# yitian97/SDformerFlow

Measured on AMD Instinct MI355X. Metric: event-frames/sec fwd (1x10x2x288x384), higher is better.
Workload: dtype f16x2; 1 GPU; BASELINE configs[1]: MS_SpikingformerFlowNet_en4 forward, batch 1 per GPU, 10-bin 288x384 voxel, neuron=lif; a step = one forward of one sample; 2 HIP streams per GPU, each replaying the HIP graph of one launch sequence that carries 10 independent batch-1 forwards of different voxels (replicas: every flow map bit-equal to a separate batch-1 forward, asserted by --full runs); one process per GPU; in_flight=2, replicas_per_launch=10, samples_in_flight=20, hip_graph=True, weight_planes=2

## Files before the change

### sdformerflow_amd/csrc/spike_conv_wres.hip

```cpp
#include "spike_mm.h"
#include "switches.h"

#ifdef SDF_STAMP
__device__ unsigned long long g_wres_stamp[32];
#define STAMP(var) var = __builtin_readcyclecounter()
#define STAMP_ADD(acc, a, b) acc += (b) - (a)
#else
#define STAMP(var)
#define STAMP_ADD(acc, a, b)
#endif

namespace sdfmm {
namespace {

constexpr int TH = 8, TW = 16;
constexpr int HH = TH + 2, HWID = TW + 2;
constexpr int NB = 32;
constexpr uint32_t INV = 0x80000000u;

typedef __attribute__((ext_vector_type(4))) uint32_t u32x4;

__device__ __forceinline__ __amdgpu_buffer_rsrc_t make_rsrc(const void* p) {
  return __builtin_amdgcn_make_buffer_rsrc(const_cast<void*>(p), 0, (int)INV, 0x00020000);
}
// ... 340 lines not shown
  static constexpr int RCH = HW8 * CIN16;
  static constexpr int CPL = (HH8 + 1) / 2;
  static_assert(RCH <= 128, "a halo row must fit the 128 lanes of a half group");
  static_assert((PS / 4) % 8 == 4 && (WP / 4) % 8 == 4, "pitches must be 4 x odd dwords");
  static_assert(S2 || CIN % 32 == 0, "stride 1: K steps of 32 must not straddle taps");
  static_assert(!S2 || RB == 1, "stride 2: one row block per wave");
  static_assert(KH == 1 || S2, "channel passes: stride-2 form only");
  static constexpr int step_off(int ks) {
    constexpr int n = CIN16;
    if (ks < 3 * n) return (ks / n) * RPB + (ks % n) * 16;
    if (ks < 4 * n) return XE * PS + (ks - 3 * n) * 16;
    return 2 * RPB + XE * PS + (ks - 4 * n) * 32;
  }
  static constexpr int step_base(int ks) { return ks < 3 * CIN16 ? 0 : (ks < 4 * CIN16 ? 1 : 2); }
  static __device__ __forceinline__ int slot(int kc) {
    constexpr int n = CIN16;
    const int tap = kc / (n * KH), cg = kc - tap * (n * KH), hf = cg / n, c = cg - hf * n, ky = tap / 3, kx = tap - 3 * ky;
    const int base = 2 * KS * hf;
    if (kx != 1) return base + 2 * (ky * n + c) + (kx >> 1);
    if (ky < 2) return base + 2 * (3 * n + c) + ky;
    return base + 2 * 4 * n + c;
  }
};

template <int TT, int CIN16, int RB, int NGRP, bool S2 = false, int KH = 1, bool SPK = false>
__global__ __launch_bounds__(256 * NGRP) void spike_conv_wres_i8_kernel(GemmParams P, const float* __restrict__ col_scale) {
  static_assert(!SPK || TT > 0, "spikes-only: a fused-neuron form");
  using G = GeoI8<CIN16, RB, S2, KH>;
  constexpr int ST = S2 ? 2 : 1;
  constexpr int CING = G::CING;
  constexpr bool EARLY = KH > 1;
  constexpr bool SPIKE = TT > 0;
  const int T = SPIKE ? P.d.sn_T : 1;
  constexpr int CIN = G::CIN, K = G::K, PS = G::PS, RPB = G::RPB, WP = G::WP, TH8 = G::TH8, TW8 = G::TW8;
  constexpr int W_BYTES = 3 * NB * WP;
  constexpr int PAR = 2 * NB * 4;
  constexpr int NT = 256 * NGRP;
  static_assert(W_BYTES + NGRP * G::HALO + PAR + 64 <= 160 * 1024, "LDS budget");
  __shared__ __attribute__((aligned(16))) uint8_t smem[W_BYTES + NGRP * G::HALO + PAR + 64];
  uint8_t* W_s = smem;
  float* par_s = reinterpret_cast<float*>(smem + W_BYTES + NGRP * G::HALO);
  uint32_t* cnt = reinterpret_cast<uint32_t*>(smem + W_BYTES + NGRP * G::HALO + PAR);

  const SdfSpikeGemmDesc& d = P.d;
  const int H = P.cv.OH, W = P.cv.OW;
  const int Hin = P.cv.H, Win = P.cv.W;
  const int tid = threadIdx.x;
  const int wave = __builtin_amdgcn_readfirstlane(tid >> 6), lane = tid & 63;
  const int grp = wave >> 2, cw = wave & 3;
  const int gl = tid & 255;
  const int N = d.N;
  const bool has_res = !SPK && !(S2 && SPIKE) && d.resid != nullptr;
  const bool memb = !SPK && (!SPIKE || d.out != nullptr);
  const int ohw = H * W;
  const int pm = SPIKE ? (int)(d.pos_inner / ohw) : 1, pso = SPIKE ? (int)(d.pos_ostride / ohw) : 0;
  const int tstep = SPIKE ? (int)(d.t_stride / ohw) : 0;
  const bool lif_fast = SPIKE && d.sn_kind == SDF_LIF && d.soft_reset != 0 && P.inv_tau != 0.f;
  const bool soft = d.soft_reset != 0;

  if (tid < 2 * NGRP) cnt[tid] = 0;

  const int tiles_x = (W + TW8 - 1) / TW8, tiles_img = tiles_x * ((H + TH8 - 1) / TH8);
  const int Gd = gridDim.x;
  int wg = blockIdx.x;
  if ((Gd & 7) == 0) wg = (wg & 7) * (Gd >> 3) + (wg >> 3);
  int t_begin, n_my;
  if (P.cb_inner) {
    const int nr = Gd / P.tiles_n, r = wg / P.tiles_n, cbw = wg - r * P.tiles_n;
    const int base = P.tiles_m / nr, rem = P.tiles_m % nr;
    t_begin = cbw * P.tiles_m + r * base + (r < rem ? r : rem);
    n_my = base + (r < rem ? 1 : 0);
  } else {
    const int nitems = P.ntiles;
    const int base = nitems / Gd, rem = nitems % Gd;
    t_begin = wg * base + (wg < rem ? wg : rem);
    n_my = base + (wg < rem ? 1 : 0);
  }

  const int hhalf = gl >> 7, hj = gl & 127;
  const bool hj_ok = hj < G::RCH;
  const int hpx = (hj_ok ? hj : 0) / CIN16, hc16 = (hj_ok ? hj : 0) - hpx * CIN16;
  const uint32_t h_lds0 = (uint32_t)(hhalf * RPB + (S2 ? (hpx & 1) * G::XE * PS + (hpx >> 1) * PS : hpx * PS) + hc16 * 16);
  const int h_rel0 = ((hhalf - 1) * Win + (hpx - 1)) * CING + hc16 * 16;
  const __amdgpu_buffer_rsrc_t A_rs = make_rsrc(d.A);
  u32x4 hreg[G::CPL];
  auto halo_load = [&](int img, int y0, int x0, int hf) __attribute__((always_inline)) {
    const uint32_t org = (uint32_t)(((img * Hin + ST * y0) * Win + ST * x0) * CING + hf * CIN) + (uint32_t)h_rel0;
    const bool xok = hj_ok && (unsigned)(ST * x0 + hpx - 1) < (unsigned)Win;
#pragma unroll
    for (int i = 0; i < G::CPL; ++i) {
      const int hy = 2 * i + hhalf;
      const bool ok = xok && hy < G::HH8 && (unsigned)(ST * y0 + hy - 1) < (unsigned)Hin;
      hreg[i] = __builtin_amdgcn_raw_buffer_load_b128(A_rs, ok ? org + (uint32_t)(2 * i * Win * CING) : INV, 0, 0);
    }
  };
  uint8_t* H_s = smem + W_BYTES + grp * G::HALO;
  auto halo_store = [&]() __attribute__((always_inline)) {
#pragma unroll
    for (int i = 0; i < G::CPL; ++i)
      if (hj_ok && 2 * i + hhalf < G::HH8) *reinterpret_cast<u32x4*>(H_s + h_lds0 + 2 * i * RPB) = hreg[i];
  };
  auto item_decode = [&](int item, int& cb, int& img0, int& y0, int& x0) __attribute__((always_inline)) {
    cb = item / P.tiles_m;
    const int rt = item - cb * P.tiles_m;
    const int im = rt / tiles_img, tl = rt - im * tiles_img;
    const int ty = tl / tiles_x, tx = tl - ty * tiles_x;
    img0 = SPIKE ? (im / pm) * pso + im % pm : im; y0 = ty * TH8; x0 = tx * TW8;
  };

  int ln = lane;
  asm volatile("" : "+v"(ln));
  const int l31 = ln & 31, lh = ln >> 5;
  const uint32_t a_lane = S2 ? (uint32_t)(2 * (2 * cw + (l31 >> 4)) * RPB + (l31 & 15) * PS)
                              : (uint32_t)((2 * RB * cw + (l31 >> 4)) * RPB + (l31 & 15) * PS + 16 * lh);
  const uint32_t a_base[3] = {a_lane + (uint32_t)(lh * PS), a_lane + (uint32_t)(lh * RPB), a_lane + (uint32_t)(lh * 16)};
  const uint32_t w_lane = (uint32_t)(l31 * WP + 16 * lh);
  const __amdgpu_buffer_rsrc_t out_rs = make_rsrc(d.out), res_rs = make_rsrc(d.resid), sp_rs = make_rsrc(d.out_spike);

  uint32_t nstep = 0;
  int seg_begin = 0;
#ifdef SDF_STAMP
  unsigned long long s0 = 0, s1 = 0, s2 = 0, s3 = 0, s4 = 0, s5 = 0, a_issue = 0, a_wait = 0, a_mfma = 0, a_epi = 0, a_hand = 0, a_wload = 0;
  const unsigned long long kstart = __builtin_readcyclecounter(), rstart = __builtin_amdgcn_s_memrealtime();
#endif
  while (seg_begin < n_my) {
    int cb, img0, y0, x0;
    item_decode(t_begin + seg_begin, cb, img0, y0, x0);
    int seg_end = (cb + 1) * P.tiles_m - t_begin;
    if (seg_end > n_my) seg_end = n_my;
    const int n0 = cb * NB;
    STAMP(s0);
    __syncthreads();
    {
      constexpr int KC16 = K / 16;
      constexpr int WCH = 3 * NB * KC16;
      const __amdgpu_buffer_rsrc_t W_rs = __builtin_amdgcn_make_buffer_rsrc(const_cast<uint16_t*>(d.Wp), 0, 3 * N * K, 0x00020000);
      constexpr int WB = 6, NBATCH = (WCH + NT * WB - 1) / (NT * WB);
      int tl = tid;
      asm volatile("" : "+v"(tl));
#pragma unroll 1
      for (int b = 0; b < NBATCH; ++b) {
        u32x4 wv[WB];
#pragma unroll
        for (int i = 0; i < WB; ++i) {
          const int c = tl + NT * (b * WB + i);
          const int cc = c < WCH ? c : 0;
          const int row = cc / KC16, kc = cc - row * KC16;
          const int dg = row / NB, n = row - dg * NB;
          wv[i] = __builtin_amdgcn_raw_buffer_load_b128(W_rs, c < WCH ? (uint32_t)((dg * N + n0 + n) * K + kc * 16) : INV, 0, 0);
        }
#pragma unroll
        for (int i = 0; i < WB; ++i) {
          const int c = tl + NT * (b * WB + i);
          const int cc = c < WCH ? c : 0;
          const int row = cc / KC16, kc = cc - row * KC16;
          if (c < WCH) *reinterpret_cast<u32x4*>(W_s + row * WP + (S2 ? G::slot(kc) : kc) * 16) = wv[i];
        }
      }
      if (S2 && (G::NP & 1) && tid < 3 * NB) {
        u32x4 z; z.x = z.y = z.z = z.w = 0u;
#pragma unroll
        for (int hf = 0; hf < KH; ++hf) *reinterpret_cast<u32x4*>(W_s + tid * WP + (2 * G::KS * hf + G::NP) * 16) = z;
      }
      if (tid < 2 * NB) {
        const int which = tid / NB, n = tid - which * NB;
        const float sc = col_scale[n0 + n];
        par_s[tid] = which == 0 ? (d.alpha ? d.alpha[n0 + n] * sc : sc) : (d.alpha ? d.beta[n0 + n] : 0.f);
      }
    }
    __syncthreads();
    STAMP(s1); STAMP_ADD(a_wload, s0, s1);

    int it = seg_begin + grp;
    if (it < seg_end) {
      item_decode(t_begin + it, cb, img0, y0, x0);
      halo_load(img0, y0, x0, 0);
      if (nstep) wait_ge(&cnt[NGRP + grp], 4 * nstep);
      halo_store();
      signal(&cnt[grp], lane);
    }
    for (; it < seg_end; it += NGRP) {
      item_decode(t_begin + it, cb, img0, y0, x0);
      float vmem[SPIKE ? 16 * RB : 1];
      if (SPIKE) {
#pragma unroll
        for (int e = 0; e < 16 * RB; ++e) vmem[e] = soft ? 0.f : d.v_reset;
      }
#pragma unroll 1
      for (int t = 0; t < T; ++t) {
        STAMP(s0);
        const int img = img0 + t * tstep;
        const uint32_t ld4 = (uint32_t)d.ldo * 4u, col4 = (uint32_t)(n0 + 4 * lh) * 4u;
        const int ybase = y0 + 2 * RB * cw + (l31 >> 4), xbase = x0 + (l31 & 15);
        const uint32_t g00 = (uint32_t)((img * H + ybase) * W + xbase);
        auto row_g = [&](int rb, int q4) __attribute__((always_inline)) -> uint32_t {
          return (ybase + 2 * rb < H && xbase < W) ? g00 + (uint32_t)(2 * rb * W) : INV;
        };
        auto rowoff = [&](int rb, int q4) __attribute__((always_inline)) -> uint32_t {
          const uint32_t g = row_g(rb, q4);
          return g != INV ? g * ld4 + col4 + (uint32_t)(32 * q4) : INV;
        };
        float4 rs[RB][4];
#pragma unroll
        for (int rb = 0; rb < RB; ++rb)
#pragma unroll
          for (int q4 = 0; q4 < 4; ++q4) rs[rb][q4] = make_float4(0.f, 0.f, 0.f, 0.f);
        auto load_res = [&]() __attribute__((always_inline)) {
#pragma unroll
          for (int rb = 0; rb < RB; ++rb)
#pragma unroll
            for (int q4 = 0; q4 < 4; ++q4) rs[rb][q4] = buf_load16f(res_rs, rowoff(rb, q4));
        };
        constexpr bool RES_EARLY = !SPIKE || RB == 1;
        if (RES_EARLY && has_res) load_res();
        bool have_next = true;
        auto request_next = [&](int hf) __attribute__((always_inline)) {
          int ni = img, ny = y0, nx = x0, nhf = hf + 1;
          if (nhf == KH) {
            nhf = 0; ni = img0 + (t + 1) * tstep;
            if (t + 1 == T) {
              if (it + NGRP < seg_end) { int ncb; item_decode(t_begin + it + NGRP, ncb, ni, ny, nx); }
              else have_next = false;
            }
          }
          if (have_next) halo_load(ni, ny, nx, nhf);
        };
        auto hand_over = [&]() __attribute__((always_inline)) {
          if (have_next) {
            wait_ge(&cnt[NGRP + grp], 4 * nstep);
            halo_store();
            signal(&cnt[grp], lane);
          }
        };

        i32x16 acc[3][RB];
#pragma unroll
        for (int dg = 0; dg < 3; ++dg)
#pragma unroll
          for (int rb = 0; rb < RB; ++rb)
#pragma unroll
            for (int e = 0; e < 16; ++e) acc[dg][rb][e] = 0;
        constexpr int KS = G::KS;
        constexpr int PF = (RB == 1 && (NGRP == 2 || SPK)) ? 2 : 1;
#pragma unroll
        for (int hf = 0; hf < KH; ++hf) {
          ++nstep;
          if (EARLY) request_next(hf);
          STAMP(s1);
          wait_ge(&cnt[grp], 4 * nstep);
          STAMP(s2);
          i32x4 fa[PF + 1][RB], fb[PF + 1][3];
          auto frag = [&](int ks, int set) __attribute__((always_inline)) {
            if constexpr (S2) {
              fa[set][0] = *reinterpret_cast<const i32x4*>(H_s + a_base[G::step_base(ks)] + G::step_off(ks));
            } else {
              constexpr int C32 = CIN / 32;
              const int tap = ks / C32, c = ks - tap * C32;
              const int ky = tap / 3, kx = tap - 3 * ky;
#pragma unroll
              for (int rb = 0; rb < RB; ++rb)
                fa[set][rb] = *reinterpret_cast<const i32x4*>(H_s + a_lane + ((2 * rb + ky) * RPB + kx * PS + c * 32));
            }
#pragma unroll
            for (int dg = 0; dg < 3; ++dg)
              fb[set][dg] = *reinterpret_cast<const i32x4*>(W_s + w_lane + (dg * NB * WP + (hf * KS + ks) * 32));
          };
#pragma unroll
          for (int i = 0; i < PF; ++i) frag(i, i);
#pragma unroll
          for (int ks = 0; ks < KS; ++ks) {
            if (ks + PF < KS) frag(ks + PF, (ks + PF) % (PF + 1));
            __builtin_amdgcn_sched_barrier(0);
#pragma unroll
            for (int dg = 0; dg < 3; ++dg)
#pragma unroll
              for (int rb = 0; rb < RB; ++rb)
                acc[dg][rb] = __builtin_amdgcn_mfma_i32_32x32x32_i8(fb[ks % (PF + 1)][dg], fa[ks % (PF + 1)][rb], acc[dg][rb], 0, 0, 0);
            __builtin_amdgcn_sched_barrier(0);
          }
          signal(&cnt[NGRP + grp], lane);
          if (EARLY && hf + 1 < KH) hand_over();
        }
        STAMP(s3);

        if (!RES_EARLY && has_res) load_res();
        if (!EARLY) request_next(KH - 1);
#pragma unroll
        for (int rb = 0; rb < RB; ++rb) {
          float4 om[4];
#pragma unroll
          for (int q4 = 0; q4 < 4; ++q4) {
            __builtin_amdgcn_sched_barrier(0);
            float v[4];
#pragma unroll
            for (int j = 0; j < 4; ++j) {
              const int e = q4 * 4 + j;
              const int lo = acc[1][rb][e] * 256 + acc[0][rb][e];
              v[j] = __builtin_fmaf((float)acc[2][rb][e], 65536.f, (float)lo);
            }
            const float4 al4 = *reinterpret_cast<const float4*>(par_s + 8 * q4 + 4 * lh);
            const float4 be4 = *reinterpret_cast<const float4*>(par_s + NB + 8 * q4 + 4 * lh);
            float4 o;
            o.x = __builtin_fmaf(v[0], al4.x, be4.x) + rs[rb][q4].x; o.y = __builtin_fmaf(v[1], al4.y, be4.y) + rs[rb][q4].y;
            o.z = __builtin_fmaf(v[2], al4.z, be4.z) + rs[rb][q4].z; o.w = __builtin_fmaf(v[3], al4.w, be4.w) + rs[rb][q4].w;
            om[q4] = o;
            if (SPIKE) {
              const float xs[4] = {o.x, o.y, o.z, o.w};
              uint32_t pk = 0;
              if (lif_fast) {
#pragma unroll
                for (int j = 0; j < 4; ++j) {
                  float& vm = vmem[rb * 16 + q4 * 4 + j];
                  const float hcur = vm + (xs[j] - vm) * P.inv_tau;
                  const float dth = hcur - d.v_th;
                  const bool fire = dth >= 0.f;
                  vm = fire ? dth : hcur;
                  pk |= fire ? (1u << (8 * j)) : 0u;
                }
              } else {
#pragma unroll
                for (int j = 0; j < 4; ++j) {
                  float& vm = vmem[rb * 16 + q4 * 4 + j];
                  const float hcur = neuron_charge(d.sn_kind == SDF_IF, vm, xs[j], d.tau, P.inv_tau, d.v_reset, soft || d.v_reset == 0.f);
                  const float sp = fire_reset(vm, hcur, d.v_th, d.v_reset, soft);
                  pk |= ((__float_as_uint(sp) >> 29) & 1u) << (8 * j);
                }
              }
              const uint32_t g = row_g(rb, q4);
              __builtin_amdgcn_raw_buffer_store_b32(pk, sp_rs, g != INV ? g * (uint32_t)N + (uint32_t)(n0 + 8 * q4 + 4 * lh) : INV, 0, 0);
            }
          }
          if (memb) {
            const bool o1 = (l31 & 1) != 0, o2 = (l31 & 2) != 0;
            qt4(om[0].x, om[1].x, om[2].x, om[3].x, o1, o2);
            qt4(om[0].y, om[1].y, om[2].y, om[3].y, o1, o2);
            qt4(om[0].z, om[1].z, om[2].z, om[3].z, o1, o2);
            qt4(om[0].w, om[1].w, om[2].w, om[3].w, o1, o2);
            const int ql = l31 & 3;
            const bool yok = ybase + 2 * rb < H;
            const uint32_t gq = g00 + (uint32_t)(2 * rb * W) - (uint32_t)ql;
#pragma unroll
            for (int j = 0; j < 4; ++j) {
              const bool ok = yok && xbase - ql + j < W;
              buf_store16f(out_rs, ok ? (gq + (uint32_t)j) * ld4 + (uint32_t)(n0 + 8 * ql + 4 * lh) * 4u : INV, om[j]);
            }
          }
        }
        STAMP(s4);
        hand_over();
        STAMP(s5);
        STAMP_ADD(a_issue, s0, s1); STAMP_ADD(a_wait, s1, s2); STAMP_ADD(a_mfma, s2, s3); STAMP_ADD(a_epi, s3, s4); STAMP_ADD(a_hand, s4, s5);
      }
    }
    seg_begin = seg_end;
  }
#ifdef SDF_STAMP
  if (blockIdx.x == 0 && (tid == 0 || tid == 256)) {
    unsigned long long* o = g_wres_stamp + (tid ? 16 : 0);
    o[0] = a_issue; o[1] = a_wait; o[2] = a_mfma; o[3] = a_epi; o[4] = a_hand; o[5] = a_wload; o[6] = nstep;
    o[7] = __builtin_readcyclecounter() - kstart; o[8] = __builtin_amdgcn_s_memrealtime() - rstart;
  }
#endif
}

template <int NSPLIT, int TT>
int launch_c(const GemmParams& P, dim3 grid, hipStream_t s) {
  switch (P.cv.Cin) {
    case 96: SDF_LAUNCH((spike_conv_wres_kernel<NSPLIT, TT, 6>), grid, dim3(512), 0, s, P); return 0;
    default: return SDF_E_SHAPE;
  }
}

}

bool spike_conv_wres_supports(const GemmParams& P, bool any_size) {
  const SdfSpikeGemmDesc& d = P.d;
  const ConvGeom& c = P.cv;
  const bool s1 = c.Cin == 96 && c.sy == 1 && c.sx == 1 && c.H == c.OH && c.W == c.OW;
  const bool s2 = (c.Cin == 48 || (c.Cin == 96 && d.sn_T == 0)) && c.sy == 2 && c.sx == 2 && c.OH == (c.H - 1) / 2 + 1 &&
                  c.OW == (c.W - 1) / 2 + 1 && d.nsplit == SDF_PLANES_I8X3 && !(d.sn_T > 0 && d.resid);
  if ((!s1 && !s2) || c.KWc != 3 || d.K != 9 * c.Cin) return false;
  if (c.dy[0] != -1 || c.dy[1] != 0 || c.dy[2] != 1 || c.dx[0] != -1 || c.dx[1] != 0 || c.dx[2] != 1) return false;
  if (d.N % NB || (d.nsplit != 1 && d.nsplit != 2 && d.nsplit != SDF_PLANES_I8X3) || d.out_rowmap || d.add || d.zg_nH > 0) return false;
  if (d.nsplit == SDF_PLANES_I8X3 && (!d.col_scale || d.bias)) return false;
  if (d.sn_T != 0 && d.sn_T != 10 && !(d.nsplit == SDF_PLANES_I8X3 && (d.sn_T == 5 || d.sn_T == 20))) return false;
  const int64_t imgs = d.M / ((int64_t)c.OH * c.OW);
  if (d.sn_T > 0) {
    if (d.sn_kind == SDF_PSN || d.bias) return false;
    if (d.nsplit != SDF_PLANES_I8X3 && !any_size) return false;
    const int64_t ohw = (int64_t)c.OH * c.OW;
    if (d.pos_inner % ohw || d.pos_ostride % ohw || d.t_stride % ohw || d.pos_count % ohw || d.t_stride == 0) return false;
    if (imgs % d.sn_T) return false;
  }
  if (d.ldo % 4 || (d.out && !sdf_aligned(d.out, 16)) || (d.resid && !sdf_aligned(d.resid, 16))) return false;
  const int64_t lim = (int64_t)1 << 31;
  if (imgs * c.H * c.W * c.Cin >= lim || d.M * d.ldo * 4 >= lim || d.M * d.N >= lim) return false;
  const int64_t tiles = imgs * ((c.OH + TH - 1) / TH) * ((c.OW + TW - 1) / TW) / (d.sn_T > 0 ? d.sn_T : 1);
  return any_size || tiles * (d.N / NB) >= 512;
}

int launch_spike_conv_wres(const GemmParams& Pin, hipStream_t s) {
  GemmParams P = Pin;
  const SdfSpikeGemmDesc& d = P.d;
  const ConvGeom& c = P.cv;
  const int64_t imgs = d.M / ((int64_t)c.OH * c.OW);
  const int T = d.sn_T > 0 ? d.sn_T : 1;
  int th = TH;
  if (d.nsplit == SDF_PLANES_I8X3) {
    const int64_t items16 = (imgs / T) * ((c.OH + 15) / 16) * ((c.OW + TW - 1) / TW) * (d.N / NB);
    const char* erb = sdf_sw(SW_CONV_WRES_RB);
    th = (c.sy == 1 && (erb ? erb[0] == '2' : items16 >= 2048)) ? 16 : 8;
  }
  P.tiles_m = (int)((imgs / T) * ((c.OH + th - 1) / th) * ((c.OW + TW - 1) / TW));
  P.tiles_n = d.N / NB;
  P.ntiles = P.tiles_m * P.tiles_n;
  P.ksplit = 1; P.spc = 0; P.partial = nullptr;
  int G = P.ntiles < 256 ? P.ntiles : 256;
  int rc;
  if (d.nsplit == SDF_PLANES_I8X3) {
    if (c.Cin != 96 && c.Cin != 48) return SDF_E_SHAPE;
    {
      const char* eg0 = sdf_sw(SW_CONV_WRES_GROUPS);
      const int ng = (d.sn_T > 0 && th == 8 && (eg0 ? eg0[0] == '3' : true)) ? 3 : 2;
      const int rounds = (P.ntiles + 256 * ng - 1) / (256 * ng), per = ng * rounds;
      if (P.ntiles >= 64) G = (P.ntiles + per - 1) / per;
      const bool cbi = [] { const char* e = sdf_sw(SW_CONV_WRES_CB_INNER); return !e || e[0] != '0'; }();
      if (cbi && P.ntiles >= 64) {
        int nr = (P.tiles_m + per - 1) / per;
        while (nr * P.tiles_n <= 256 && (nr * P.tiles_n) % 8) ++nr;
        const int g2 = nr * P.tiles_n;
        if (g2 <= 256 && g2 % 8 == 0) { G = g2; P.cb_inner = 1; }
      }
    }
    const char* eg = sdf_sw(SW_CONV_WRES_GROUPS);
    const bool g3 = d.sn_T > 0 && th == 8 && (eg ? eg[0] == '3' : true);
    const dim3 grid((unsigned)G);
// ... 76 lines not shown
```

### sdformerflow_amd/csrc/spike_gemm.hip

```cpp
#include "wide_common.h"
#include "switches.h"
#include <stdlib.h>

namespace {
using namespace sdfmm;

constexpr int KC = 96;
constexpr int A_LD = KC + 8;
constexpr int W_LD = KC + 8;

template <int NSPLIT, int NB, int RB, int TT, int WAVES, bool CONV>
__global__ __launch_bounds__(64 * WAVES) void spike_gemm_kernel(GemmParams P) {
  constexpr bool SPIKE = TT > 0;
  constexpr int T = SPIKE ? TT : 1;
  constexpr int NT = 64 * WAVES;
  constexpr int BM = 32 * RB * WAVES, BN = 32 * NB, WR = 32 * RB;
  constexpr int NPOS = (16 * RB) / T;
  constexpr int A_CH = BM * (KC / 16);
  constexpr int AIT = A_CH / NT;
  constexpr int WCH = NSPLIT * BN * (KC / 8);
  constexpr int WIT = (WCH + NT - 1) / NT;
  static_assert(!SPIKE || NPOS >= 1, "T does not fit the accumulator slots of one lane");
  __shared__ __attribute__((aligned(16))) uint8_t smem[BM * A_LD + NSPLIT * BN * W_LD * 2];
  uint8_t* A_s = smem;
// ... 462 lines not shown
    const bool legal = d->N % 96 == 0 && spike_mm_pp_supports(P, false);
    bool use_pp = legal && ((spike && (d->sn_T == 10 || d->sn_T == 20)) ||
                           (!spike && ((d->K >= 384 && d->M >= 32768) || d->K >= 2048 || (d->K >= 384 && d->N >= 864))));
    if (e && e[0] == '0') use_pp = false;
    if (e && e[0] == '2') use_pp = legal;
    if (use_pp) return launch_spike_mm_pp(P, false, sdf_stream(stream));
  }
  if (!ok(cfg)) return SDF_E_SHAPE;
  const int nb = CFG_NB[cfg], rb = CFG_RB[cfg], waves = CFG_WAVES[cfg];
  const int npos = spike ? (16 * rb) / d->sn_T : 0;
  P.tiles_m = (int)(spike ? (d->pos_count + 2 * waves * npos - 1) / (2 * waves * npos)
                          : (d->M + 32 * rb * waves - 1) / (32 * rb * waves));
  P.tiles_n = (d->N + 32 * nb - 1) / (32 * nb);
  P.ntiles = P.tiles_m * P.tiles_n;
  const size_t lds = (size_t)32 * rb * waves * A_LD + (size_t)d->nsplit * 32 * nb * W_LD * 2;
  int wg_per_cu = lds > 80 * 1024 ? 1 : (lds > 53 * 1024 ? 2 : 3);
  if (const char* e = sdf_sw(SW_GEMM_WGS)) { const int v = atoi(e); if (v >= 1 && v <= 8) wg_per_cu = v; }
  const int G = P.ntiles < 256 * wg_per_cu ? P.ntiles : 256 * wg_per_cu;
  dim3 grid((unsigned)G);
  hipStream_t s = sdf_stream(stream);
  const int rc = d->nsplit == 1 ? launch_cfg<1>(P, cfg, grid, s) : (d->nsplit == 2 ? launch_cfg<2>(P, cfg, grid, s) : launch_cfg<3>(P, cfg, grid, s));
  if (rc) return rc;
  SDF_LAUNCH_CHECK();
  return 0;
}

static int conv2d_build(const SdfSpikeConvDesc* c, GemmParams& P, bool& i8x3, bool& tiled) {
  if (!c) return SDF_E_NULL;
  const SdfSpikeGemmDesc* d = &c->g;
  if (!d->A || !d->Wp) return SDF_E_NULL;
  const bool spike = d->sn_T > 0;
  if (spike ? !d->out_spike : !d->out) return SDF_E_NULL;
  if (c->H < 1 || c->W < 1 || c->H > 32767 || c->W > 32767 || c->OH < 1 || c->OW < 1) return SDF_E_SHAPE;
  if (c->Cin < 48 || c->Cin % 16 || c->KH < 1 || c->KH > 3 || c->KW < 1 || c->KW > 3 || c->sy < 1 || c->sx < 1) return SDF_E_SHAPE;
  if (d->K != c->KH * c->KW * c->Cin || d->N % 32 || d->M % ((int64_t)c->OH * c->OW) || d->M >= (1LL << 31)) return SDF_E_SHAPE;
  if ((d->M / ((int64_t)c->OH * c->OW)) * c->H * c->W >= (1LL << 31)) return SDF_E_SHAPE;
  tiled = d->nsplit == SDF_PLANES_I8X3_TILED;
  i8x3 = d->nsplit == SDF_PLANES_I8X3 || tiled;
  if (!i8x3 && (d->nsplit < 1 || d->nsplit > 3)) return SDF_E_DTYPE;
  if (!i8x3 && !sdf_scale_ok(d)) return SDF_E_DTYPE;
  if (i8x3 && !d->col_scale) return SDF_E_NULL;
  if (d->alpha && !d->beta) return SDF_E_NULL;
  if (d->zg_nH > 0) return SDF_E_SHAPE;
  P.d = *d;
  P.d.lda = 0;
  P.inv_tau = 0.f;
  P.acc_scale = i8x3 ? 1.f : sdf_acc_scale(d);
  if (spike) {
    if ((d->sn_T != 10 && !(i8x3 && (d->sn_T == 5 || d->sn_T == 20))) || d->pos_count < 1 || d->pos_inner < 1 ||
        d->pos_count * d->sn_T != d->M) return SDF_E_SHAPE;
    if (d->sn_kind != SDF_LIF && d->sn_kind != SDF_PSN && d->sn_kind != SDF_IF) return SDF_E_DTYPE;
    if (d->sn_kind == SDF_PSN && (!d->psn_w || !d->psn_b)) return SDF_E_NULL;
    if (!sdf_tau_ok(d->sn_kind, d->tau)) return SDF_E_SHAPE;
    if (d->out_rowmap || d->bias || d->add) return SDF_E_SHAPE;
    if (d->resid && !d->out) return SDF_E_NULL;
    if (d->out && (d->ldo < d->N || !sdf_aligned(d->out, 4))) return SDF_E_SHAPE;
    if (!sdf_aligned(d->out_spike, 16)) return SDF_E_ALIGN;
    P.inv_tau = sdf_inv_tau(d->sn_kind, d->tau);
  }
  if (!sdf_aligned(d->A, 16) || !sdf_aligned(d->Wp, 16)) return SDF_E_ALIGN;
  ConvGeom& cv = P.cv;
  cv.H = c->H; cv.W = c->W; cv.Cin = c->Cin; cv.OH = c->OH; cv.OW = c->OW; cv.sy = c->sy; cv.sx = c->sx;
  cv.KWc = c->KW;
  cv.kw_mul = c->KW == 1 ? 32 : (c->KW == 2 ? 16 : 11);
  for (int i = 0; i < 3; ++i) { cv.dy[i] = c->dy[i]; cv.dx[i] = c->dx[i]; }
  return 0;
}

extern "C" int sdf_spike_deconv3x3s2_fwd(const SdfSpikeDeconvDesc* d, void* stream) {
  if (!d) return SDF_E_NULL;
  if (!d->spikes || !d->digits || !d->cscale || !d->out) return SDF_E_NULL;
  if ((d->alpha != nullptr) != (d->beta != nullptr)) return SDF_E_NULL;
  if (d->imgs < 1 || d->H < 1 || d->W < 1 || (d->T != 10 && d->T != 20) || d->imgs % d->T) return SDF_E_SHAPE;
  if (d->Cin < 16 || d->Cin % 16 || 4 * d->Cin > 1024 || d->Cout < 8 || d->Cout % 8) return SDF_E_SHAPE;
  const int64_t rows = (int64_t)d->imgs * d->H * d->W;
  if (rows * d->Cin >= (1LL << 31) || rows * 4 * d->Cout * 4 >= (1LL << 31)) return SDF_E_SHAPE;
  if (!sdf_aligned(d->spikes, 16) || !sdf_aligned(d->digits, 16) || !sdf_aligned(d->out, 16)) return SDF_E_ALIGN;
  if (spike_deconv_wres_supports(d->imgs, d->H, d->W, d->Cin, d->Cout))
    return launch_spike_deconv_wres(d->spikes, d->digits, d->cscale, d->alpha, d->beta, d->out, d->imgs, d->H, d->W, d->Cout, sdf_stream(stream));
  WidePmParams P = {};
  P.A = d->spikes; P.W = d->digits; P.cscale = d->cscale; P.N = 4 * d->Cout; P.K = 4 * d->Cin;
  P.HW = d->H * d->W; P.P = (int64_t)(d->imgs / d->T) * P.HW;
  P.alpha = d->alpha; P.beta = d->beta; P.x = d->out; P.ldo = d->Cout; P.no_resid = 1;
  P.cv_H = d->H; P.cv_W = d->W; P.cv_Cin = d->Cin; P.dc_cout = d->Cout;
  P.res_stage = 1;
  if (!res_pm_takes(P, d->T, 2)) return SDF_E_SHAPE;
  return launch_res_pm(P, d->T, 2, sdf_stream(stream));
}

extern "C" int sdf_spike_conv2d_fwd(const SdfSpikeConvDesc* c, void* stream) {
  GemmParams P;
  bool i8x3 = false, tiled = false;
  {
    const int rc = conv2d_build(c, P, i8x3, tiled);
    if (rc) return rc;
  }
  const SdfSpikeGemmDesc* d = &c->g;
  const bool spike = d->sn_T > 0;
  if (i8x3 && wide_conv_supports(P)) return launch_wide_conv(P, sdf_stream(stream));
  if (i8x3 && smallm_conv_supports(P)) return launch_smallm_conv(P, sdf_stream(stream));
  if (tiled) return SDF_E_SHAPE;
  const char* ewr = sdf_sw(SW_CONV_WRES);
  if (!(ewr && ewr[0] == '0') && spike_conv_wres_supports(P, i8x3 || (ewr && ewr[0] == '2'))) return launch_spike_conv_wres(P, sdf_stream(stream));
  if (i8x3) return SDF_E_SHAPE;
  if (spike_mm_pp_supports(P, true)) return launch_spike_mm_pp(P, true, sdf_stream(stream));
  const int64_t imgs = d->M / ((int64_t)c->OH * c->OW);
  if (!spike && imgs > 1) {
// ... 73 lines not shown
```

### sdformerflow_amd/engine.py

```python
from __future__ import annotations

import torch
import torch.nn.functional as F

from . import hip
from .STSwinNet_SNN.Spiking_swin_transformer3D import get_window_size, merge_row_map, window_slice_map

BN_EPS = 1e-5
_WIDE_MINC = 96


def bn_affine(bn, device):
    w, b = bn.weight.detach().float().cpu(), bn.bias.detach().float().cpu()
    m, v = bn.running_mean.detach().float().cpu(), bn.running_var.detach().float().cpu()
    alpha = w * torch.rsqrt(v + BN_EPS)
    beta = (b.double() - m.double() * alpha.double()).float()
    return alpha.contiguous().to(device), beta.contiguous().to(device)


class _Lin:

    def __init__(self, linear, bn, device, nsplit, digits=True):
        w = linear.weight.detach().float().to(device).contiguous()
        self.N, self.K = w.shape
# ... 182 lines not shown
            self.preds.append((hip.split_weight(wp, ns), bp, _np(p.sn, dev), w2.shape[0], w2.to(dev).contiguous(),
                               p.conv[0].bias.detach().float().to(dev).contiguous()))

    def _slice_map(self, B, D, H, W, ws, ss):
        key = ("win", B, D, H, W, ws, ss, self.replicas)
        if key not in self._maps:
            if self.replicas and B > 1:
                m1, nW = self._slice_map_1(D, H, W, ws, ss)
                if nW % ws[0]:
                    raise hip.ReplicaGeometryError(f"replicas need a window count per sample ({nW}) that is a multiple of the window depth ({ws[0]})")
                self._maps[key] = (hip.replica_slice_map(m1, nW, B, ws[0], ws[1] * ws[2], D * H * W), B * nW)
            else:
                self._maps[key] = hip.window_slice_map(B, D, H, W, ws, ss, self.device)
        return self._maps[key]

    def _slice_map_1(self, D, H, W, ws, ss):
        key = ("win", 1, D, H, W, ws, ss, False)
        if key not in self._maps:
            self._maps[key] = hip.window_slice_map(1, D, H, W, ws, ss, self.device)
        return self._maps[key]

    def _merge_map(self, B, D, H, W):
        key = ("merge", B, D, H, W)
        if key not in self._maps:
            src, H2, W2 = merge_row_map(B, D, H, W)
            out_map = None
            if B > 1:
                t = torch.arange(D).view(D, 1, 1)
                b = torch.arange(B).view(1, B, 1)
                p = torch.arange(H2 * W2).view(1, 1, -1)
                out_map = ((b * D + t) * (H2 * W2) + p).reshape(-1).to(torch.int32).to(self.device)
            self._maps[key] = (torch.from_numpy(src.reshape(-1)).to(self.device), H2, W2, out_map)
        return self._maps[key]

    @staticmethod
    def _check_cl(x):
        if x.dim() != 5 or not x.is_contiguous() or x.dtype != torch.float32:
            raise hip.SdfError(f"expected a contiguous fp32 (B,D,h,w,C) tensor, got shape {tuple(x.shape)} strides {x.stride()} "
                               f"{x.dtype}; call .contiguous() (the update is in place)")

    def _rec(self, name, spikes, layout):
        if self.tape is not None:
            self.tape.append((name, spikes.clone(), layout))

    def _neuron_bd(self, x, p, bn=None, out_dtype=torch.uint8):
        self._check_cl(x)
        B, D, h, w, Cc = x.shape
        out = torch.empty(x.shape, dtype=out_dtype, device=x.device)
        a, b = bn if bn is not None else (None, None)
        n = h * w * Cc
        hip.neuron_fwd(x, out, D, B, n, D * n, n, D * n, n, p, alpha=a, beta=b, Cch=Cc, inner=1)
        return out

    def _conv3x3(self, s, Wp, Cout, stride=1, bn=None, resid=None, sn=None, membrane=False, _dst=None):
        B, D, h, w, Cin = s.shape
        oh, ow = (h + 2 - 3) // stride + 1, (w + 2 - 3) // stride + 1
        a, b = bn if bn is not None else (None, None)
        digits = getattr(Wp, "digits", None)
        if self.replicas and B > 1 and _dst is None and digits is None:
            return self._conv3x3_chunks(s, Wp, Cout, stride, bn, resid, sn, membrane, 1)
        if self.replicas and B > 1 and _dst is None and digits is not None:
            route = lambda n: (hip.smallm_conv_applicable(n * D, h, w, Cin, Cout, stride, D), hip.conv_wres_applicable(n * D, h, w, Cin, Cout, stride, 1),
                               hip.conv_wres_applicable(n * D, h, w, Cin, Cout, stride, D))
            r1 = route(1)
            if route(B) != r1:
                bc = max(n for n in range(1, B) if B % n == 0 and route(n) == r1)
                return self._conv3x3_chunks(s, Wp, Cout, stride, bn, resid, sn, membrane, bc)
        if digits is not None and (sn is None or sn.kind in ("lif", "if", "psn")) and hip.smallm_conv_applicable(B * D, h, w, Cin, Cout, stride, D):
            out = None if sn is not None and not membrane else torch.empty((B, D, oh, ow, Cout), dtype=torch.float32, device=s.device)
            sp = torch.empty((B, D, oh, ow, Cout), dtype=torch.uint8, device=s.device) if sn is not None else None
            try:
                hip.spike_conv2d(s, digits, B * D, h, w, Cin, oh, ow, 3, 3, stride, (-1, 0, 1), (-1, 0, 1), out=out, out_spike=sp, alpha=a, beta=b,
                                 resid=resid if (membrane or sn is None) else None, sn=sn, sn_T=D if sn is not None else 0,
                                 pos=(B * oh * ow, oh * ow, D * oh * ow, oh * ow))
                return sp if sn is not None and not membrane else ((out, sp) if sn is not None else out)
            except hip.SdfError as e:
                if e.rc not in (hip.E_SHAPE, hip.E_ALIGN):
                    raise
                if sn is not None and sn.kind == "psn":
                    m = torch.empty((B, D, oh, ow, Cout), dtype=torch.float32, device=s.device)
                    hip.spike_conv2d(s, Wp, B * D, h, w, Cin, oh, ow, 3, 3, stride, (-1, 0, 1), (-1, 0, 1), out=m, alpha=a, beta=b,
                                     resid=resid if membrane else None)
                    sp = self._neuron_bd(m, sn)
                    return (m, sp) if membrane else sp
        if digits is not None and B > 1 and not hip.conv_wres_applicable(B * D, h, w, Cin, Cout, stride, 1):
            bc = self._digit_chunk(B, D, h, w, Cin, Cout, stride)
            if bc:
                return self._conv3x3_chunks(s, Wp, Cout, stride, bn, resid, sn, membrane, bc)
        if digits is not None and sn is not None and (sn.kind == "psn" or D not in (5, 10, 20)) and \
                hip.conv_wres_applicable(B * D, h, w, Cin, Cout, stride, 1):
            m = self._conv3x3(s, Wp, Cout, stride, bn=bn, resid=resid if membrane else None)
            sp = self._neuron_bd(m, sn)
            return (m, sp) if membrane else sp
        if digits is not None and (sn is None or (sn.kind != "psn" and D in (5, 10, 20))) and \
                hip.conv_wres_applicable(B * D, h, w, Cin, Cout, stride, D if sn is not None else 1):
            Wp = digits
        if sn is None:
            out = _dst[0] if _dst is not None and len(_dst) == 1 and _dst[0].dtype == torch.float32 else \
                torch.empty((B, D, oh, ow, Cout), dtype=torch.float32, device=s.device)
            hip.spike_conv2d(s, Wp, B * D, h, w, Cin, oh, ow, 3, 3, stride, (-1, 0, 1), (-1, 0, 1), out=out, alpha=a, beta=b,
                             resid=resid)
            return out
        if _dst is not None and len(_dst) == (2 if membrane else 1) and _dst[-1].dtype == torch.uint8:
            out, m = _dst[-1], (_dst[0] if membrane else None)
        else:
            out = torch.empty((B, D, oh, ow, Cout), dtype=torch.uint8, device=s.device)
            m = torch.empty((B, D, oh, ow, Cout), dtype=torch.float32, device=s.device) if membrane else None
        hip.spike_conv2d(s, Wp, B * D, h, w, Cin, oh, ow, 3, 3, stride, (-1, 0, 1), (-1, 0, 1), out=m, out_spike=out, alpha=a, beta=b,
                         resid=resid if membrane else None, sn=sn, sn_T=D, pos=(B * oh * ow, oh * ow, D * oh * ow, oh * ow))
        return (m, out) if membrane else out

    def _conv3x3_chunks(self, s, Wp, Cout, stride, bn, resid, sn, membrane, bc):
        B, D, h, w, _ = s.shape
        oh, ow = (h + 2 - 3) // stride + 1, (w + 2 - 3) // stride + 1
        kinds = [torch.float32] if sn is None else ([torch.float32, torch.uint8] if membrane else [torch.uint8])
        outs = tuple(torch.empty((B, D, oh, ow, Cout), dtype=k, device=s.device) for k in kinds)
        if resid is not None:
            resid = resid.view(B, D, oh, ow, Cout)
        for b0 in range(0, B, bc):
            dst = tuple(o[b0:b0 + bc] for o in outs)
            r = self._conv3x3(s[b0:b0 + bc], Wp, Cout, stride, bn, None if resid is None else resid[b0:b0 + bc], sn, membrane, dst)
            r = r if isinstance(r, tuple) else (r,)
            for o, t in zip(dst, r):
                if t.data_ptr() != o.data_ptr():
                    o.copy_(t)
        return outs if len(outs) > 1 else outs[0]

    def _rb(self, B):
        return 1 if self.replicas else B

    @staticmethod
    def _digit_chunk(B, D, h, w, Cin, Cout, stride):
        for bc in range(B - 1, 0, -1):
            if B % bc == 0 and hip.conv_wres_applicable(bc * D, h, w, Cin, Cout, stride, 1):
                return bc
        return 0

    @staticmethod
    def _fusable(B, D, h, w, C, Wp=None):
        big = (B * D * h * w + 255) // 256 * (C // 96) >= 128
        if D == 10:
            return big
        if not (big and D in (5, 20) and C == 96 and getattr(Wp, "digits", None) is not None and Wp.shape[-1] == 9 * 96):
            return False
        bc = B if hip.conv_wres_applicable(B * D, h, w, 96, C, 1, 1) else MSFlowEngine._digit_chunk(B, D, h, w, 96, C, 1)
        return bc > 0 and hip.conv_wres_applicable(bc * D, h, w, 96, C, 1, D)

    def _resblock(self, m, rb, s1=None, next_sn=None):
        B, D, h, w, _ = m.shape
        if s1 is None:
            s1 = self._neuron_bd(m, rb.sn1)
        self._rec(rb.name + "sn1.spiking_neuron.", s1, "BDHWC->TBCHW")
        fus = self._fusable(self._rb(B), D, h, w, rb.C, rb.w1) or \
            (getattr(rb.w1, "digits", None) is not None and rb.sn2.kind in ("lif", "if", "psn") and hip.smallm_conv_applicable(self._rb(B) * D, h, w, rb.C, rb.C, 1, D))
        if fus:
            s2 = self._conv3x3(s1, rb.w1, rb.C, bn=rb.bn1, sn=rb.sn2)
        else:
            s2 = self._neuron_bd(self._conv3x3(s1, rb.w1, rb.C), rb.sn2, bn=rb.bn1)
        self._rec(rb.name + "sn2.spiking_neuron.", s2, "BDHWC->TBCHW")
        if next_sn is not None and fus:
            return self._conv3x3(s2, rb.w2, rb.C, bn=rb.bn2, resid=m, sn=next_sn, membrane=True)
        m2 = self._conv3x3(s2, rb.w2, rb.C, bn=rb.bn2, resid=m)
        return (m2, self._neuron_bd(m2, next_sn)) if next_sn is not None else m2

    def patch_embed(self, x):
        xv = x
        if x.size(1) > self.num_bins:
            x = x[:, :self.num_bins]
        B, T = x.shape[0], self.num_steps
        H, W = x.shape[-2:]
        num_ch = self.num_bins * 2 // T
        if hip.head_conv_sn_supported(T, H, W, num_ch, self.head_w_oihw.shape[0]) and xv.is_contiguous():
            s = hip.head_conv_sn(xv, self.head_w_oihw, B, T, H, W, self.head_sn, alpha=self.head_bn[0], beta=self.head_bn[1],
                                 voxel_bins=xv.shape[1])
        else:
            ev = x.permute(0, 2, 3, 4, 1)
            xr = torch.stack([ev[:, i % 2, :, :, (i // 2) * T:(i // 2 + 1) * T] for i in range(num_ch)], -1)
            xr = xr.permute(0, 3, 1, 2, 4).contiguous().view(B * T, H, W, num_ch)
            y = F.conv2d(xr.permute(0, 3, 1, 2), self.head_w, None, 1, 1).contiguous(memory_format=torch.channels_last)
            s = self._neuron_bd(y.permute(0, 2, 3, 1).view(B, T, H, W, -1), self.head_sn, bn=self.head_bn)
        self._rec(self.pe_name + "head.sn.spiking_neuron.", s, "BDHWC->TBCHW")
        sns = [rb.sn1 for rb in self.pe_res] + [self.proj_sn]
        C0 = self.conv_w.shape[1]
        oh, ow = (H - 1) // 2 + 1, (W - 1) // 2 + 1
        fus = self._fusable(self._rb(B), T, oh, ow, C0)
        if not fus and T in (5, 20) and getattr(self.conv_w, "digits", None) is not None and sns[0].kind != "psn":
            c0 = s.shape[-1]
            Br = self._rb(B)
            bc = Br if hip.conv_wres_applicable(Br * T, H, W, c0, C0, 2, 1) else self._digit_chunk(Br, T, H, W, c0, C0, 2)
            fus = bc > 0 and hip.conv_wres_applicable(bc * T, H, W, c0, C0, 2, T)
        if fus:
            m, s1 = self._conv3x3(s, self.conv_w, C0, stride=2, bn=self.conv_bn, sn=sns[0], membrane=True)
        else:
            m = self._conv3x3(s, self.conv_w, C0, stride=2, bn=self.conv_bn)
            s1 = self._neuron_bd(m, sns[0])
        for i, rb in enumerate(self.pe_res):
            m, s1 = self._resblock(m, rb, s1=s1, next_sn=sns[i + 1])
        Bm, Dm, h, w, Cc = m.shape
        self._rec(self.pe_name + "proj.sn.spiking_neuron.", s1, "BDHWC->TBCHW")
        if hip.pointwise_conv_supported(Cc, self.proj_res_w2.shape[0]):
            res = hip.pointwise_conv_f32(m.view(B * T, h, w, Cc), self.proj_res_w2, 2, self.proj_res_b)
        else:
            res = F.conv2d(m.view(B * T, h, w, Cc).permute(0, 3, 1, 2), self.proj_res_w, self.proj_res_b, 2)
            res = res.contiguous(memory_format=torch.channels_last).permute(0, 2, 3, 1)
        return self._conv3x3(s1, self.proj_w, self.proj_w.shape[1], stride=2, bn=self.proj_bn, resid=res)

    def _zsrc_map(self, rowmap, B_, Tq, N1, nH, x_rows, key):
        key = ("zsrc", nH, self.replicas) + key
        if key not in self._maps:
            B = key[3]
            if self.replicas and B > 1:
                _, D, H, W, ws, ss = key[3:]
                m1, nW = self._slice_map_1(D, H, W, ws, ss)
                z1 = hip.window_zsrc_map(m1, nW, Tq, N1, nH, x_rows // B)
                self._maps[key] = hip.replica_zsrc_map(z1, nW, B, Tq, N1, nH * 32)
            else:
                self._maps[key] = hip.window_zsrc_map(rowmap, B_, Tq, N1, nH, x_rows)
        return self._maps[key]

    def attention(self, x, blk: _Block, score_out=None, emit=None):
        self._check_cl(x)
        B, D, H, W, Cc = x.shape
        ws, ss = get_window_size((D, H, W), blk.window_size, blk.shift_size)
        if tuple(ws) != tuple(blk.window_size):
            raise hip.SdfError(f"feature map {(D, H, W)} is smaller than the window {tuple(blk.window_size)}: the positional encoding of "
                               "Spiking_QK_WindowAttention3D is defined for the nominal window only (reference Spiking_swin_transformer3D.py:678)")
        rowmap, B_ = self._slice_map(B, D, H, W, ws, ss)
        Tq, N1 = ws[0], ws[1] * ws[2]
        rep_windows = B_ // B if self.replicas and B > 1 else 0
        if rep_windows and (self.tape is not None or score_out is not None):
            raise hip.SdfError("the parity tape and log=True follow one forward: run them without replicas")
        keep = [] if score_out is not None else None
        if self.tape is not None:
            rows, keep = B_ * N1, []
            xs = torch.empty((Tq, rows, Cc), dtype=torch.uint8, device=x.device)
            hip.neuron_fwd(x, xs, Tq, 1, rows * Cc, 0, 0, 0, rows * Cc, blk.sn_proj, rowmap=rowmap, rowlen=Cc)
            self._rec(blk.name + "attn.proj_sn.spiking_neuron.", xs, "flat")
        info = {}
        zsrc = self._zsrc_map(rowmap, B_, Tq, N1, blk.nH, B * D * H * W, (B, D, H, W, tuple(ws), tuple(ss))) if Cc >= _WIDE_MINC and Tq == 2 else None
        kw = dict(qk=blk.qk) if blk.qk is not None else dict(q_lin=blk.q, k_lin=blk.k, pe=blk.pe)
        hip.qk_attn(x, rowmap, B_, Tq, N1, blk.nH, blk.p, blk.sn_proj, blk.sn_q, blk.sn_k, blk.sn2_q, keep_ws=keep, x_src=zsrc, emit=emit,
                    info=info, rep_windows=rep_windows, **kw)
        if score_out is not None:
            e = keep[0][:Tq * B_ * N1 * Cc].view(Tq, B_ * N1, Cc)
            score_out.append(attention_score(e, blk.attn_sn, blk.nH, Tq, B_, N1).view(Tq, B_, ws[1], ws[2], Cc))
        if keep and self.tape is not None:
            M = Tq * B_ * N1
            qk = keep[0][(M * Cc + 255) // 256 * 256:][:M * 2 * Cc]
            q, k = (qk.view(M, 2 * Cc)[:, :Cc], qk.view(M, 2 * Cc)[:, Cc:]) if blk.qk is not None else (qk[:M * Cc], qk[M * Cc:])
            self._rec(blk.name + "attn.sn_q.spiking_neuron.", q.reshape(Tq, B_ * N1, Cc), "flat")
            self._rec(blk.name + "attn.sn_k.spiking_neuron.", k.reshape(Tq, B_ * N1, Cc), "flat")
        self._emitted = bool(info.get("emitted"))
        return x
# ... 287 lines not shown
```

Measured before the change: 834.1 samples/s.

## Store only even-position membrane rows from last patch-embed resblock via rowmap

The last patch-embed resblock conv now writes its f32 membrane output only at even (y,x) positions, through a row map into a quarter-size buffer, because the next consumer is a stride-2 pointwise conv. The pointwise conv then runs with stride 1 on the compacted tensor. This cuts membrane store bandwidth and the strided read in the residual projection. The residual loads in the spiking path are also split so part is issued before the MMA loop. It adds a rowmap load and DPP shuffles in the epilogue, and the rowmap path in the kernel becomes valid only under specific planes and sn_T conditions.

```diff
diff --git a/sdformerflow_amd/csrc/spike_conv_wres.hip b/sdformerflow_amd/csrc/spike_conv_wres.hip
--- a/sdformerflow_amd/csrc/spike_conv_wres.hip
+++ b/sdformerflow_amd/csrc/spike_conv_wres.hip
@@ -416,6 +416,8 @@
   const int N = d.N;
   const bool has_res = !SPK && !(S2 && SPIKE) && d.resid != nullptr;
   const bool memb = !SPK && (!SPIKE || d.out != nullptr);
+  constexpr bool MAPPED = SPIKE && !SPK && !S2;
+  const bool has_map = MAPPED && memb && d.out_rowmap != nullptr;
   const int ohw = H * W;
   const int pm = SPIKE ? (int)(d.pos_inner / ohw) : 1, pso = SPIKE ? (int)(d.pos_ostride / ohw) : 0;
   const int tstep = SPIKE ? (int)(d.t_stride / ohw) : 0;
@@ -479,7 +481,9 @@
                               : (uint32_t)((2 * RB * cw + (l31 >> 4)) * RPB + (l31 & 15) * PS + 16 * lh);
   const uint32_t a_base[3] = {a_lane + (uint32_t)(lh * PS), a_lane + (uint32_t)(lh * RPB), a_lane + (uint32_t)(lh * 16)};
   const uint32_t w_lane = (uint32_t)(l31 * WP + 16 * lh);
-  const __amdgpu_buffer_rsrc_t out_rs = make_rsrc(d.out), res_rs = make_rsrc(d.resid), sp_rs = make_rsrc(d.out_spike);
+  const __amdgpu_buffer_rsrc_t out_rs = has_map ? __builtin_amdgcn_make_buffer_rsrc(d.out, 0, (int)(d.out_rows * d.ldo * 4), 0x00020000) : make_rsrc(d.out);
+  const __amdgpu_buffer_rsrc_t res_rs = make_rsrc(d.resid), sp_rs = make_rsrc(d.out_spike);
+  const __amdgpu_buffer_rsrc_t map_rs = __builtin_amdgcn_make_buffer_rsrc(const_cast<int32_t*>(d.out_rowmap), 0, has_map ? (int)(d.M * 4) : 0, 0x00020000);
 
   uint32_t nstep = 0;
   int seg_begin = 0;
@@ -569,14 +573,20 @@
         for (int rb = 0; rb < RB; ++rb)
 #pragma unroll
           for (int q4 = 0; q4 < 4; ++q4) rs[rb][q4] = make_float4(0.f, 0.f, 0.f, 0.f);
-        auto load_res = [&]() __attribute__((always_inline)) {
-#pragma unroll
-          for (int rb = 0; rb < RB; ++rb)
-#pragma unroll
-            for (int q4 = 0; q4 < 4; ++q4) rs[rb][q4] = buf_load16f(res_rs, rowoff(rb, q4));
+        auto load_res = [&](int rb, int qa = 0, int qb = 4) __attribute__((always_inline)) {
+#pragma unroll
+          for (int q4 = qa; q4 < qb; ++q4) rs[rb][q4] = buf_load16f(res_rs, rowoff(rb, q4));
         };
-        constexpr bool RES_EARLY = !SPIKE || RB == 1;
-        if (RES_EARLY && has_res) load_res();
+        constexpr bool RES_SPLIT = SPIKE && RB > 1;
+        constexpr int RES_Q0 = 2;
+        if (has_res) {
+          if (RES_SPLIT) load_res(0, 0, RES_Q0);
+          else {
+#pragma unroll
+            for (int rb = 0; rb < RB; ++rb) load_res(rb);
+          }
+        }
+        int32_t mrow[MAPPED ? RB : 1];
         bool have_next = true;
         auto request_next = [&](int hf) __attribute__((always_inline)) {
           int ni = img, ny = y0, nx = x0, nhf = hf + 1;
@@ -647,7 +657,19 @@
         }
         STAMP(s3);
 
-        if (!RES_EARLY && has_res) load_res();
+        if (RES_SPLIT && has_res) {
+          load_res(0, RES_Q0, 4);
+#pragma unroll
+          for (int rb = 1; rb < RB; ++rb) load_res(rb);
+        }
+        if (MAPPED && has_map) {
+#pragma unroll
+          for (int rb = 0; rb < RB; ++rb) {
+            const uint32_t g = row_g(rb, 0);
+            const int32_t v = (int32_t)__builtin_amdgcn_raw_buffer_load_b32(map_rs, g != INV ? g * 4u : INV, 0, 0);
+            mrow[rb] = g != INV ? v : -1;
+          }
+        }
         if (!EARLY) request_next(KH - 1);
 #pragma unroll
         for (int rb = 0; rb < RB; ++rb) {
@@ -703,10 +725,20 @@
             const int ql = l31 & 3;
             const bool yok = ybase + 2 * rb < H;
             const uint32_t gq = g00 + (uint32_t)(2 * rb * W) - (uint32_t)ql;
-#pragma unroll
-            for (int j = 0; j < 4; ++j) {
-              const bool ok = yok && xbase - ql + j < W;
-              buf_store16f(out_rs, ok ? (gq + (uint32_t)j) * ld4 + (uint32_t)(n0 + 8 * ql + 4 * lh) * 4u : INV, om[j]);
+            const uint32_t colq = (uint32_t)(n0 + 8 * ql + 4 * lh) * 4u;
+            if (MAPPED && has_map) {
+              const int32_t m0 = __builtin_amdgcn_mov_dpp(mrow[MAPPED ? rb : 0], 0x00, 0xF, 0xF, true), m1 = __builtin_amdgcn_mov_dpp(mrow[MAPPED ? rb : 0], 0x55, 0xF, 0xF, true);
+              const int32_t m2 = __builtin_amdgcn_mov_dpp(mrow[MAPPED ? rb : 0], 0xAA, 0xF, 0xF, true), m3 = __builtin_amdgcn_mov_dpp(mrow[MAPPED ? rb : 0], 0xFF, 0xF, 0xF, true);
+              const int32_t mj[4] = {m0, m1, m2, m3};
+#pragma unroll
+              for (int j = 0; j < 4; ++j)
+                if (mj[j] >= 0) buf_store16f(out_rs, (uint32_t)mj[j] * ld4 + colq, om[j]);
+            } else {
+#pragma unroll
+              for (int j = 0; j < 4; ++j) {
+                const bool ok = yok && xbase - ql + j < W;
+                buf_store16f(out_rs, ok ? (gq + (uint32_t)j) * ld4 + colq : INV, om[j]);
+              }
             }
           }
         }
@@ -745,7 +777,8 @@
                   c.OW == (c.W - 1) / 2 + 1 && d.nsplit == SDF_PLANES_I8X3 && !(d.sn_T > 0 && d.resid);
   if ((!s1 && !s2) || c.KWc != 3 || d.K != 9 * c.Cin) return false;
   if (c.dy[0] != -1 || c.dy[1] != 0 || c.dy[2] != 1 || c.dx[0] != -1 || c.dx[1] != 0 || c.dx[2] != 1) return false;
-  if (d.N % NB || (d.nsplit != 1 && d.nsplit != 2 && d.nsplit != SDF_PLANES_I8X3) || d.out_rowmap || d.add || d.zg_nH > 0) return false;
+  if (d.N % NB || (d.nsplit != 1 && d.nsplit != 2 && d.nsplit != SDF_PLANES_I8X3) || d.add || d.zg_nH > 0) return false;
+  if (d.out_rowmap && !(d.nsplit == SDF_PLANES_I8X3 && s1 && d.sn_T > 0 && d.out && d.out_rows > 0 && d.out_rows * d.ldo * 4 < ((int64_t)1 << 31))) return false;
   if (d.nsplit == SDF_PLANES_I8X3 && (!d.col_scale || d.bias)) return false;
   if (d.sn_T != 0 && d.sn_T != 10 && !(d.nsplit == SDF_PLANES_I8X3 && (d.sn_T == 5 || d.sn_T == 20))) return false;
   const int64_t imgs = d.M / ((int64_t)c.OH * c.OW);
diff --git a/sdformerflow_amd/csrc/spike_gemm.hip b/sdformerflow_amd/csrc/spike_gemm.hip
--- a/sdformerflow_amd/csrc/spike_gemm.hip
+++ b/sdformerflow_amd/csrc/spike_gemm.hip
@@ -538,7 +538,7 @@
     if (d->sn_kind != SDF_LIF && d->sn_kind != SDF_PSN && d->sn_kind != SDF_IF) return SDF_E_DTYPE;
     if (d->sn_kind == SDF_PSN && (!d->psn_w || !d->psn_b)) return SDF_E_NULL;
     if (!sdf_tau_ok(d->sn_kind, d->tau)) return SDF_E_SHAPE;
-    if (d->out_rowmap || d->bias || d->add) return SDF_E_SHAPE;
+    if ((d->out_rowmap && !(i8x3 && !tiled && d->out)) || d->bias || d->add) return SDF_E_SHAPE;
     if (d->resid && !d->out) return SDF_E_NULL;
     if (d->out && (d->ldo < d->N || !sdf_aligned(d->out, 4))) return SDF_E_SHAPE;
     if (!sdf_aligned(d->out_spike, 16)) return SDF_E_ALIGN;
diff --git a/sdformerflow_amd/engine.py b/sdformerflow_amd/engine.py
--- a/sdformerflow_amd/engine.py
+++ b/sdformerflow_amd/engine.py
@@ -258,7 +258,7 @@
         hip.neuron_fwd(x, out, D, B, n, D * n, n, D * n, n, p, alpha=a, beta=b, Cch=Cc, inner=1)
         return out
 
-    def _conv3x3(self, s, Wp, Cout, stride=1, bn=None, resid=None, sn=None, membrane=False, _dst=None):
+    def _conv3x3(self, s, Wp, Cout, stride=1, bn=None, resid=None, sn=None, membrane=False, _dst=None, even_only=False):
         B, D, h, w, Cin = s.shape
         oh, ow = (h + 2 - 3) // stride + 1, (w + 2 - 3) // stride + 1
         a, b = bn if bn is not None else (None, None)
@@ -312,9 +312,23 @@
         else:
             out = torch.empty((B, D, oh, ow, Cout), dtype=torch.uint8, device=s.device)
             m = torch.empty((B, D, oh, ow, Cout), dtype=torch.float32, device=s.device) if membrane else None
+        rowmap = None
+        if even_only and membrane and _dst is None and Wp is digits and stride == 1 and hip.sw("SDF_PE_EVEN_STORE") != "0":
+            m = torch.empty((B, D, (oh + 1) // 2, (ow + 1) // 2, Cout), dtype=torch.float32, device=s.device)
+            rowmap = self._even_map(B * D, oh, ow, s.device)
         hip.spike_conv2d(s, Wp, B * D, h, w, Cin, oh, ow, 3, 3, stride, (-1, 0, 1), (-1, 0, 1), out=m, out_spike=out, alpha=a, beta=b,
-                         resid=resid if membrane else None, sn=sn, sn_T=D, pos=(B * oh * ow, oh * ow, D * oh * ow, oh * ow))
+                         resid=resid if membrane else None, out_rowmap=rowmap, sn=sn, sn_T=D,
+                         pos=(B * oh * ow, oh * ow, D * oh * ow, oh * ow))
         return (m, out) if membrane else out
+
+    def _even_map(self, imgs, oh, ow, dev):
+        key = ("even", imgs, oh, ow)
+        if key not in self._maps:
+            h2, w2 = (oh + 1) // 2, (ow + 1) // 2
+            y, x = torch.arange(oh, device=dev).view(1, oh, 1), torch.arange(ow, device=dev).view(1, 1, ow)
+            r = (torch.arange(imgs, device=dev).view(imgs, 1, 1) * h2 + y // 2) * w2 + x // 2
+            self._maps[key] = torch.where((y % 2 == 0) & (x % 2 == 0), r, -1).to(torch.int32).reshape(-1).contiguous()
+        return self._maps[key]
 
     def _conv3x3_chunks(self, s, Wp, Cout, stride, bn, resid, sn, membrane, bc):
         B, D, h, w, _ = s.shape
@@ -352,7 +366,7 @@
         bc = B if hip.conv_wres_applicable(B * D, h, w, 96, C, 1, 1) else MSFlowEngine._digit_chunk(B, D, h, w, 96, C, 1)
         return bc > 0 and hip.conv_wres_applicable(bc * D, h, w, 96, C, 1, D)
 
-    def _resblock(self, m, rb, s1=None, next_sn=None):
+    def _resblock(self, m, rb, s1=None, next_sn=None, even_only=False):
         B, D, h, w, _ = m.shape
         if s1 is None:
             s1 = self._neuron_bd(m, rb.sn1)
@@ -365,7 +379,7 @@
             s2 = self._neuron_bd(self._conv3x3(s1, rb.w1, rb.C), rb.sn2, bn=rb.bn1)
         self._rec(rb.name + "sn2.spiking_neuron.", s2, "BDHWC->TBCHW")
         if next_sn is not None and fus:
-            return self._conv3x3(s2, rb.w2, rb.C, bn=rb.bn2, resid=m, sn=next_sn, membrane=True)
+            return self._conv3x3(s2, rb.w2, rb.C, bn=rb.bn2, resid=m, sn=next_sn, membrane=True, even_only=even_only)
         m2 = self._conv3x3(s2, rb.w2, rb.C, bn=rb.bn2, resid=m)
         return (m2, self._neuron_bd(m2, next_sn)) if next_sn is not None else m2
 
@@ -400,11 +414,14 @@
         else:
             m = self._conv3x3(s, self.conv_w, C0, stride=2, bn=self.conv_bn)
             s1 = self._neuron_bd(m, sns[0])
+        pw = hip.pointwise_conv_supported(self.pe_res[-1].C, self.proj_res_w2.shape[0]) if self.pe_res else False
         for i, rb in enumerate(self.pe_res):
-            m, s1 = self._resblock(m, rb, s1=s1, next_sn=sns[i + 1])
+            m, s1 = self._resblock(m, rb, s1=s1, next_sn=sns[i + 1], even_only=pw and i == len(self.pe_res) - 1)
         Bm, Dm, h, w, Cc = m.shape
         self._rec(self.pe_name + "proj.sn.spiking_neuron.", s1, "BDHWC->TBCHW")
-        if hip.pointwise_conv_supported(Cc, self.proj_res_w2.shape[0]):
+        if m.shape[2:4] != s1.shape[2:4]:
+            res = hip.pointwise_conv_f32(m.view(B * T, h, w, Cc), self.proj_res_w2, 1, self.proj_res_b)
+        elif hip.pointwise_conv_supported(Cc, self.proj_res_w2.shape[0]):
             res = hip.pointwise_conv_f32(m.view(B * T, h, w, Cc), self.proj_res_w2, 2, self.proj_res_b)
         else:
             res = F.conv2d(m.view(B * T, h, w, Cc).permute(0, 3, 1, 2), self.proj_res_w, self.proj_res_b, 2)
```

Result: no change. 838.3 samples/s, median of 6 (+0.5%).
